# vymv/PupilOptixLab

Hardware: AMD Instinct MI355X
Metric: Mrays/sec + ms/frame, 1M-tri scene @1920x1080 8spp; 1/2/4/8-GPU scaling (higher is better)
Workload: dtype f32; 1 GPU; config4: 1,000,014-primitive sphere field (1,000,014 tris), 1920x1080, 8 spp, max_depth 4; rays_traced_plain_process=18645769168, parallelism=tiles32x1, area_emitters=2, accel=flat, emitter_select=guide, bvh_nodes=213019

## Files before the change

include/pupil_pt.h:

```cpp
#pragma once
#include <stddef.h>
#include <stdint.h>

#ifdef __cplusplus
extern "C" {
#endif

#define PUPIL_OK 0
#define PUPIL_ERR_INVALID -1
#define PUPIL_ERR_HIP -2
#define PUPIL_ERR_OOM -3
#define PUPIL_ERR_IO -4
#define PUPIL_ERR_UNSUPPORTED -5

#define PUPIL_TEX_RGB 0u
#define PUPIL_TEX_BITMAP 1u
#define PUPIL_TEX_CHECKERBOARD 2u

#define PUPIL_MAT_UNKNOWN 0u
#define PUPIL_MAT_DIFFUSE 1u
#define PUPIL_MAT_DIELECTRIC 2u
#define PUPIL_MAT_ROUGH_DIELECTRIC 3u
#define PUPIL_MAT_CONDUCTOR 4u
#define PUPIL_MAT_ROUGH_CONDUCTOR 5u
// ... 266 lines not shown
int pupil_debug_math(int device, uint32_t n, const float *x, const float *y2, float *out);
int pupil_debug_select_emitter(pupil_pt *pt, uint32_t n, const float *p, int32_t *out);
int pupil_debug_read_emitters(pupil_pt *pt, uint32_t first, uint32_t n, float *out);
int pupil_debug_emitter_sample(pupil_pt *pt, uint32_t emitter, uint32_t n, const float *xi, const float *pos_nrm,
                               float *out);
int pupil_debug_read_emitter_guide(pupil_pt *pt, uint32_t *bits, uint32_t *guide, uint32_t *inout_count);
int pupil_debug_shade_tables(pupil_pt *pt, uint32_t caps[4], uint32_t *fit);
int pupil_debug_env(pupil_pt *pt, uint32_t n, const float *xi_or_dir, const float *pos_nrm, uint32_t mode, float *out);
int pupil_debug_read_env_tables(pupil_pt *pt, uint32_t *width, uint32_t *height, float *col_cdf, float *row_cdf,
                                float *row_weight, float *normalization);
int pupil_debug_tex_sample(pupil_pt *pt, uint32_t material, uint32_t slot, uint32_t n, const float *uv, float *out);
int pupil_debug_read_material(pupil_pt *pt, uint32_t material, uint32_t *type, float out[3]);
int pupil_debug_fill_tlas_reserve(pupil_pt *pt, float value);
int pupil_debug_bvh_reinsert(int device, uint32_t n, const float *boxes, uint32_t rounds, double *cost,
                             uint32_t *kept, uint32_t *rejected);
int pupil_debug_partition(int device, uint32_t n, uint32_t capacity, const uint8_t *keys, uint32_t nbins,
                          uint32_t mode, uint32_t shift_or_tag, uint32_t bin_mask, const uint64_t *cum_in,
                          uint32_t *out, uint32_t *counts, uint32_t *starts, uint32_t *total, uint32_t *log,
                          uint64_t *cum_out, uint64_t *snap, uint32_t *info);

enum { PUPIL_IMAGE_AUTO = 0, PUPIL_IMAGE_EXR = 1, PUPIL_IMAGE_HDR = 2, PUPIL_IMAGE_PFM = 3 };
int pupil_image_save(const char *path, uint32_t width, uint32_t height, const float *rgba, uint32_t format);

int pupil_image_load(const char *path, uint32_t *width, uint32_t *height, float *rgba);

enum {
    PUPIL_DENOISE_USE_ALBEDO = 1,
    PUPIL_DENOISE_USE_NORMAL = 1 << 1,
    PUPIL_DENOISE_APPLY_TO_AOV = 1 << 2,
    PUPIL_DENOISE_USE_TEMPORAL = 1 << 3,
// ... 57 lines not shown
```

pupiloptixlab_amd/abi.py:

```python
from __future__ import annotations

import ctypes as C
import os

TEX_RGB, TEX_BITMAP, TEX_CHECKERBOARD = 0, 1, 2
MAT_UNKNOWN, MAT_DIFFUSE, MAT_DIELECTRIC, MAT_ROUGH_DIELECTRIC = 0, 1, 2, 3
MAT_CONDUCTOR, MAT_ROUGH_CONDUCTOR, MAT_PLASTIC, MAT_ROUGH_PLASTIC = 4, 5, 6, 7
EMITTER_NONE, EMITTER_TRI_AREA, EMITTER_SPHERE, EMITTER_CONST_ENV, EMITTER_ENV_MAP = 0, 1, 2, 3, 4
EMITTER_POINT, EMITTER_SPOT, EMITTER_DIRECTIONAL = 5, 6, 7
SHAPE_MESH, SHAPE_SPHERE = 0, 1

PUPIL_OK = OK = 0
ERR_INVALID, ERR_HIP, ERR_OOM, ERR_IO, ERR_UNSUPPORTED = -1, -2, -3, -4, -5
VERTS_DEVICE, VERTS_REBUILD = 1, 2
IMAGE_AUTO, IMAGE_EXR, IMAGE_HDR, IMAGE_PFM = 0, 1, 2, 3
ERR_NAMES = {-1: "PUPIL_ERR_INVALID", -2: "PUPIL_ERR_HIP", -3: "PUPIL_ERR_OOM", -4: "PUPIL_ERR_IO",
             -5: "PUPIL_ERR_UNSUPPORTED"}

f32p = C.POINTER(C.c_float)
u32p = C.POINTER(C.c_uint32)


class Texture(C.Structure):
    _fields_ = [("type", C.c_uint32), ("c0", C.c_float * 3), ("c1", C.c_float * 3),
# ... 155 lines not shown
                                           C.c_uint32, C.c_uint32, C.c_void_p]),
    "pupil_pt_query_rays": (C.c_int, [C.c_void_p, C.c_uint32, C.c_void_p, C.c_uint32, C.POINTER(RayHits), C.c_void_p]),
    "pupil_pt_query_camera": (C.c_int, [C.c_void_p, C.c_float, C.c_float, C.c_uint32, C.c_uint32, C.c_uint32,
                                         C.c_uint32, C.c_void_p, C.POINTER(RayHits), C.c_void_p]),
    "pupil_pt_query_info": (C.c_int, [C.c_void_p, C.POINTER(C.c_uint64), C.POINTER(C.c_uint64),
                                       C.POINTER(C.c_uint64), C.POINTER(C.c_double)]),
    "pupil_pt_radiance_rays": (C.c_int, [C.c_void_p, C.c_uint32, C.c_void_p, C.c_void_p, C.POINTER(Launch),
                                          C.POINTER(RayRadiance), C.c_void_p]),
    "pupil_pt_radiance_info": (C.c_int, [C.c_void_p, C.POINTER(C.c_uint64), C.POINTER(C.c_uint64),
                                          C.POINTER(C.c_uint64), C.POINTER(C.c_uint64), C.POINTER(C.c_uint64),
                                          C.POINTER(C.c_double)]),
    "pupil_pt_trace_rays": (C.c_int, [C.c_void_p, C.c_uint32, f32p, f32p, C.c_int]),
    "pupil_pt_export_bvh4": (C.c_int, [C.c_void_p, u32p, C.c_void_p, u32p, f32p, C.POINTER(C.c_int32)]),
    "pupil_debug_math": (C.c_int, [C.c_int, C.c_uint32, f32p, f32p, f32p]),
    "pupil_debug_bvh_reinsert": (C.c_int, [C.c_int, C.c_uint32, f32p, C.c_uint32, C.POINTER(C.c_double), u32p, u32p]),
    "pupil_debug_partition": (C.c_int, [C.c_int, C.c_uint32, C.c_uint32, C.POINTER(C.c_uint8), C.c_uint32, C.c_uint32,
                                         C.c_uint32, C.c_uint32, C.POINTER(C.c_uint64), u32p, u32p, u32p, u32p, u32p,
                                         C.POINTER(C.c_uint64), C.POINTER(C.c_uint64), u32p]),
    "pupil_image_save": (C.c_int, [C.c_char_p, C.c_uint32, C.c_uint32, f32p, C.c_uint32]),
    "pupil_debug_select_emitter": (C.c_int, [C.c_void_p, C.c_uint32, f32p, C.POINTER(C.c_int32)]),
    "pupil_debug_env": (C.c_int, [C.c_void_p, C.c_uint32, f32p, f32p, C.c_uint32, f32p]),
    "pupil_debug_emitter_sample": (C.c_int, [C.c_void_p, C.c_uint32, C.c_uint32, f32p, f32p, f32p]),
    "pupil_debug_tex_sample": (C.c_int, [C.c_void_p, C.c_uint32, C.c_uint32, C.c_uint32, f32p, f32p]),
    "pupil_image_load": (C.c_int, [C.c_char_p, C.POINTER(C.c_uint32), C.POINTER(C.c_uint32), f32p]),
    "pupil_world_create": (C.c_int, [C.POINTER(C.c_void_p)]),
    "pupil_world_load_xml": (C.c_int, [C.c_void_p, C.c_char_p]),
    "pupil_world_set_film": (C.c_int, [C.c_void_p, C.c_uint32, C.c_uint32, C.c_uint32]),
    "pupil_world_set_sensor": (C.c_int, [C.c_void_p, C.c_float, C.c_char, C.c_float, C.c_float, f32p]),
    "pupil_world_add_mesh": (C.c_int, [C.c_void_p, C.c_uint32, C.c_uint32, f32p, f32p, f32p, u32p, u32p]),
    "pupil_world_add_builtin_shape": (C.c_int, [C.c_void_p, C.c_char_p, u32p]),
# ... 72 lines not shown
```

pupiloptixlab_amd/csrc/bvh_build.hip:

```cpp
#include "bvh_build_detail.h"

#include <algorithm>
#include <cstdlib>
#include <cstring>

namespace pupil {

using namespace bvh;

namespace {

__global__ void k_prim_setup(BvhBuildInput in, float4 *recs, Aabb *boxes) {
    const uint32_t i = blockIdx.x * blockDim.x + threadIdx.x;
    if (i >= in.num_prims) return;
    const uint32_t inst_id = in.prim_inst[i];
    const DevInstance &inst = in.instances[inst_id];
    const uint32_t mtype = in.materials[inst.material].type;
    const uint32_t bin = (mtype >= 1u && mtype <= 7u) ? mtype : 8u;
    Aabb b;
    if (inst.kind == PUPIL_SHAPE_SPHERE) {
        const float *m = inst.to_world;
        const vec3 c = v3(m[3], m[7], m[11]);
        const float ex = sqrtf(m[0] * m[0] + m[1] * m[1] + m[2] * m[2]) * 1.001f;
        const float ey = sqrtf(m[4] * m[4] + m[5] * m[5] + m[6] * m[6]) * 1.001f;
// ... 90 lines not shown
__global__ void k_leaf_slots(Bvh4Node *nodes, uint32_t m, const unsigned long long *first_slot, uint32_t *slot) {
    const uint32_t j = blockIdx.x * blockDim.x + threadIdx.x;
    if (j >= m) return;
    Bvh4Node nd = nodes[j];
    for (int k = 0; k < 4; k++) {
        const int l = nd.child[k];
        if (l == kEmptyLink || l >= 0) continue;
        const uint32_t f = leaf_first(l), c = leaf_count(l), fs = (uint32_t)first_slot[f];
        for (uint32_t q = 0; q < c; q++) slot[f + q] = fs + q;
        nd.child[k] = make_leaf(fs, c);
    }
    nodes[j] = nd;
}

constexpr int kReinsDefault = 2;

BuildOptions read_build_options(uint32_t leaf_size) {
    BuildOptions o;
    const char *e = std::getenv("PUPIL_BVH_BUILDER");
    if (e && std::strcmp(e, "lbvh") == 0) o.builder = BuildOptions::Builder::Karras;
    e = std::getenv("PUPIL_BVH4_COLLAPSE");
    if (e && std::strcmp(e, "parity") == 0) o.collapse = BuildOptions::Collapse::Parity;
    else if (e && std::strcmp(e, "greedy") == 0) o.collapse = BuildOptions::Collapse::Greedy;
    o.sah_leaf = leaf_size;
    if ((e = std::getenv("PUPIL_SAH_LEAF"))) o.sah_leaf = (uint32_t)std::min(8, std::max((int)leaf_size, std::atoi(e)));
    o.reinsert_rounds = kReinsDefault;
    if ((e = std::getenv("PUPIL_BVH_REINSERT"))) o.reinsert_rounds = std::min(64, std::max(0, std::atoi(e)));
    o.reinsert_log = std::getenv("PUPIL_BVH_REINSERT_LOG") != nullptr;
    return o;
}

hipError_t leaf_slots_and_records(const BvhBuildInput &in, const uint32_t *order, const float4 *recs, bool leaf_root,
                                  BvhBuildOutput &out, hipStream_t s) {
    const uint32_t nrec = in.num_prims;
    const uint32_t g = (nrec + kBlock - 1) / kBlock;
    hipError_t err = hipSuccess;
    auto slot = scratch<uint32_t>(err, nrec);
    auto lsz = scratch<unsigned long long>(err, nrec);
    auto ssum = scratch<unsigned long long>(err, scan64_blocks((int)nrec));
    auto stot = scratch<unsigned long long>(err, 1);
    if (err) return err;
    const uint32_t m = leaf_root ? 0u : out.num_nodes4;
// ... 106 lines not shown
    float ms = 0.f;
    (void)hipEventElapsedTime(&ms, e0, e1);
    if (build_ms) *build_ms = ms;
    (void)hipEventDestroy(e0);
    (void)hipEventDestroy(e1);
    return err == hipSuccess ? 0 : -2;
}

int build_bvh4_over_boxes(const float *h_boxes, uint32_t n, std::vector<Bvh4Node> &nodes, std::vector<uint32_t> &order,
                          uint32_t *depth, hipStream_t s, int rounds, ReinsertLog *log) {
    if (n < 2) return -1;
    BuildOptions opts = read_build_options(1u);
    opts.builder = BuildOptions::Builder::Ploc;
    opts.collapse = BuildOptions::Collapse::Sah;
    if (rounds >= 0) opts.reinsert_rounds = rounds;
    const int m = (int)n;
    hipError_t err = hipSuccess;
    FrontEnd fe(err, m, false);
    Collapsed c4;
    if (!err) err = hipMemcpyAsync(fe.boxes.get(), h_boxes, sizeof(Aabb) * n, hipMemcpyHostToDevice, s);
    if (!err) {
        morton_order(fe, m, s);
        err = binary_tree(fe, m, opts, s, log);
    }
    if (!err) err = collapse_bvh4(fe.tree(m), 1u, opts, fe.spare_keys, fe.spare_vals, s, c4);
    if (!err) {
        nodes.resize(c4.num_nodes4);
        order.resize(n);
        err = hipMemcpyAsync(nodes.data(), c4.nodes4.get(), sizeof(Bvh4Node) * c4.num_nodes4, hipMemcpyDeviceToHost, s);
        if (!err) err = hipMemcpyAsync(order.data(), fe.sorted_vals, sizeof(uint32_t) * n, hipMemcpyDeviceToHost, s);
// ... 27 lines not shown
```

pupiloptixlab_amd/csrc/bvh_build_detail.h:

```cpp
#pragma once
#include <hip/hip_runtime.h>

#include <cstdint>
#include <vector>

#include "bvh4_quant.h"
#include "host/scoped_buffer.h"
#include "pt_kernels.h"

namespace pupil::bvh {

constexpr int kBlock = 256;
inline dim3 grid_for(int m) { return dim3((unsigned)((m + kBlock - 1) / kBlock)); }

struct Aabb {
    float lo[3];
    float hi[3];
};

__device__ __forceinline__ Aabb merge(const Aabb &a, const Aabb &b) {
    Aabb r;
    for (int k = 0; k < 3; k++) {
        r.lo[k] = fminf(a.lo[k], b.lo[k]);
        r.hi[k] = fmaxf(a.hi[k], b.hi[k]);
// ... 15 lines not shown

template <typename T>
DevBuf<T> scratch(hipError_t &err, size_t count) {
    DevBuf<T> b;
    if (!err) err = b.alloc(count);
    return b;
}

struct BuildOptions {
    enum class Builder { Ploc, Karras };
    enum class Collapse { Sah, Greedy, Parity };
    Builder builder = Builder::Ploc;
    Collapse collapse = Collapse::Sah;
    uint32_t sah_leaf = 0;
    int reinsert_rounds = 0;
    bool reinsert_log = false;
};

constexpr int kScanBlock = 1024;
constexpr int kScanItems = 4;
constexpr int kScanPer = kScanBlock * kScanItems;
inline int scan64_blocks(int n) { return (n + kScanPer - 1) / kScanPer; }
hipError_t scan64(unsigned long long *data, int n, unsigned long long *sums, unsigned long long *total,
                  hipStream_t s, unsigned long long *host_total = nullptr);

void scan32(uint32_t *data, uint32_t count, hipStream_t s);

struct BinaryTree;
struct FrontEnd {
    DevBuf<Aabb> boxes, node_boxes;
// ... 36 lines not shown
```

pupiloptixlab_amd/csrc/bvh_reinsert.hip:

```cpp
#include "bvh_build_detail.h"

#include <cstdio>

namespace pupil::bvh {

namespace {

constexpr int kReinsStack = 32;
constexpr int kReinsVisits = 256;

__device__ __forceinline__ int ref_u(int r, int nm1) { return r >= 0 ? r : nm1 + ~r; }
__device__ __forceinline__ int u_ref(int u, int nm1) { return u < nm1 ? u : ~(u - nm1); }

__global__ void k_reins_init(int n, const uint32_t *sorted_vals, const Aabb *prim_boxes, const int2 *node_child,
                             Aabb *box, int *parent) {
    const int i = blockIdx.x * blockDim.x + threadIdx.x;
    const int nm1 = n - 1;
    if (i < n) box[nm1 + i] = prim_boxes[sorted_vals[i]];
    if (i < nm1) {
        const int2 c = node_child[i];
        parent[ref_u(c.x, nm1)] = i;
        parent[ref_u(c.y, nm1)] = i;
        if (i == n - 2) parent[i] = -1;
    }
}

__global__ __launch_bounds__(kBlock) void k_reins_search(int n, const int2 *node_child, const Aabb *box,
                                                         const int *parent, int *cand_x, int *cand_pivot,
                                                         float *cand_gain, unsigned long long *claim) {
    const int u = blockIdx.x * blockDim.x + threadIdx.x;
    const int nm1 = n - 1, total = 2 * n - 1;
    if (u >= total) return;
    cand_x[u] = -1;
    const int P = parent[u];
    if (P < 0 || parent[P] < 0) return;
    const Aabb bl = box[u];
    const float al = half_area(bl);
    int st_node[kReinsStack];
    float st_ind[kReinsStack];
    float best = 0.f;
    int best_x = -1, best_pivot = -1;
    int visits = 0;
    int pivot = P, from = u;
    float bound = half_area(box[P]);
    Aabb shr;
    bool have_shr = false;
    while (visits < kReinsVisits) {
// ... 39 lines not shown
    if (best_x < 0) return;
    const int2 pc = node_child[P];
    const int S = ref_u(pc.x, nm1) == u ? ref_u(pc.y, nm1) : ref_u(pc.x, nm1);
    if (best_x == S) return;
    cand_x[u] = best_x;
    cand_pivot[u] = best_pivot;
    cand_gain[u] = best;
    const unsigned long long key = ((unsigned long long)__float_as_uint(best) << 32) | (unsigned)u;
    atomicMax(&claim[u], key);
    atomicMax(&claim[P], key);
    atomicMax(&claim[S], key);
    atomicMax(&claim[best_x], key);
    atomicMax(&claim[parent[best_x]], key);
}

__global__ void k_reins_resolve(int n, const int2 *node_child, const int *parent, const int *cand_x,
                                const float *cand_gain, const unsigned long long *claim, uint8_t *mover) {
    const int u = blockIdx.x * blockDim.x + threadIdx.x;
    const int nm1 = n - 1;
    if (u >= 2 * n - 1) return;
    const int X = cand_x[u];
    bool win = false;
    if (X >= 0) {
        const int P = parent[u];
        const int2 pc = node_child[P];
        const int S = ref_u(pc.x, nm1) == u ? ref_u(pc.y, nm1) : ref_u(pc.x, nm1);
        const unsigned long long key = ((unsigned long long)__float_as_uint(cand_gain[u]) << 32) | (unsigned)u;
        win = claim[u] == key && claim[P] == key && claim[S] == key && claim[X] == key && claim[parent[X]] == key;
    }
    mover[u] = win ? 1 : 0;
}

__global__ void k_reins_filter(int n, const int2 *node_child, const int *parent, const int *cand_x,
                               const int *cand_pivot, const uint8_t *mover, int3 *moves, int *num_moves) {
    const int u = blockIdx.x * blockDim.x + threadIdx.x;
    const int nm1 = n - 1;
    if (u >= 2 * n - 1 || !mover[u]) return;
    const int X = cand_x[u], pivot = cand_pivot[u];
    int a = parent[X];
    for (int k = 0; k < n && a >= 0 && a != pivot; k++) {
        if (mover[a]) return;
        a = parent[a];
    }
    const int P = parent[u], G = parent[P], XP = parent[X];
    const int sg = ref_u(node_child[G].x, nm1) == P ? 0 : 1;
    const int sx = ref_u(node_child[XP].x, nm1) == X ? 0 : 1;
    moves[atomicAdd(num_moves, 1)] = make_int3(u, sg, sx);
}

__global__ void k_reins_apply(int n, int num_moves, const int3 *moves, const int *cand_x, int2 *node_child,
                              int *parent) {
    const int k = blockIdx.x * blockDim.x + threadIdx.x;
    const int nm1 = n - 1;
    if (k >= num_moves) return;
    const int3 mv = moves[k];
    const int L = mv.x, X = cand_x[L];
    const int P = parent[L], G = parent[P], XP = parent[X];
    const int2 pc = node_child[P];
    const int S = ref_u(pc.x, nm1) == L ? ref_u(pc.y, nm1) : ref_u(pc.x, nm1);
    ((int *)&node_child[G])[mv.y] = u_ref(S, nm1);
    ((int *)&node_child[XP])[mv.z] = u_ref(P, nm1);
    node_child[P] = make_int2(u_ref(X, nm1), u_ref(L, nm1));
    parent[S] = G;
    parent[P] = XP;
    parent[X] = P;
}

__global__ void k_reins_refit(int n, const int2 *node_child, const int *parent, Aabb *box, int *node_count,
                              uint32_t *flags) {
    const int i = blockIdx.x * blockDim.x + threadIdx.x;
    const int nm1 = n - 1;
    if (i >= n) return;
    int node = parent[nm1 + i];
    for (int k = 0; k < n && node >= 0; k++) {
        __builtin_amdgcn_fence(__ATOMIC_RELEASE, "agent");
        const uint32_t prev = __hip_atomic_fetch_add(&flags[node], 1u, __ATOMIC_RELAXED, __HIP_MEMORY_SCOPE_AGENT);
        if (prev == 0u) return;
        __builtin_amdgcn_fence(__ATOMIC_ACQUIRE, "agent");
        const int2 c = node_child[node];
        box[node] = merge(box[ref_u(c.x, nm1)], box[ref_u(c.y, nm1)]);
        node_count[node] = (c.x >= 0 ? node_count[c.x] : 1) + (c.y >= 0 ? node_count[c.y] : 1);
        node = parent[node];
    }
}

__global__ __launch_bounds__(kBlock) void k_reins_cost(int m, const Aabb *box, double *partial) {
    __shared__ double sh[kBlock];
    const int i = blockIdx.x * kBlock + threadIdx.x;
    sh[threadIdx.x] = i < m ? (double)half_area(box[i]) : 0.0;
    __syncthreads();
    for (int o = kBlock / 2; o > 0; o >>= 1) {
        if ((int)threadIdx.x < o) sh[threadIdx.x] += sh[threadIdx.x + o];
        __syncthreads();
    }
    if (threadIdx.x == 0) partial[blockIdx.x] = sh[0];
}

struct ReinsertScratch {
    DevBuf<int2> w_child;
    DevBuf<Aabb> w_box;
    DevBuf<int> w_count, parent, cand_x, cand_pivot;
    DevBuf<float> cand_gain;
    DevBuf<unsigned long long> claim;
    DevBuf<uint8_t> mover;
    DevBuf<int3> moves;
    DevBuf<int> num_moves;
    DevBuf<uint32_t> flags;
    DevBuf<double> partial;
    std::vector<double> host_partial;

    ReinsertScratch(hipError_t &err, int n) {
        const int total = 2 * n - 1, nblk = (n - 1 + kBlock - 1) / kBlock;
        w_child = scratch<int2>(err, n);
        w_box = scratch<Aabb>(err, total);
        w_count = scratch<int>(err, n);
        parent = scratch<int>(err, total);
        cand_x = scratch<int>(err, total);
        cand_pivot = scratch<int>(err, total);
        cand_gain = scratch<float>(err, total);
        claim = scratch<unsigned long long>(err, total);
        mover = scratch<uint8_t>(err, total);
        moves = scratch<int3>(err, total);
        num_moves = scratch<int>(err, 1);
        flags = scratch<uint32_t>(err, n);
        partial = scratch<double>(err, nblk);
        host_partial.resize((size_t)nblk);
    }

    hipError_t cost(int n, hipStream_t s, double *out) {
        const int nblk = (int)host_partial.size();
        hipLaunchKernelGGL(k_reins_cost, dim3(nblk), dim3(kBlock), 0, s, n - 1, w_box.get(), partial.get());
        hipError_t e = hipMemcpyAsync(host_partial.data(), partial.get(), sizeof(double) * nblk, hipMemcpyDeviceToHost, s);
        if (!e) e = hipStreamSynchronize(s);
        double c = 0.0;
        for (double v : host_partial) c += v;
        *out = c;
        return e;
    }

    hipError_t round(int n, hipStream_t s, bool *moved, double *after) {
        const int total = 2 * n - 1;
        *moved = false;
        hipError_t err = hipMemsetAsync(claim.get(), 0, sizeof(unsigned long long) * total, s);
        if (!err) err = hipMemsetAsync(num_moves.get(), 0, sizeof(int), s);
        if (err) return err;
        hipLaunchKernelGGL(k_reins_search, grid_for(total), dim3(kBlock), 0, s, n, w_child.get(), w_box.get(),
                           parent.get(), cand_x.get(), cand_pivot.get(), cand_gain.get(), claim.get());
        hipLaunchKernelGGL(k_reins_resolve, grid_for(total), dim3(kBlock), 0, s, n, w_child.get(), parent.get(),
                           cand_x.get(), cand_gain.get(), claim.get(), mover.get());
        hipLaunchKernelGGL(k_reins_filter, grid_for(total), dim3(kBlock), 0, s, n, w_child.get(), parent.get(),
                           cand_x.get(), cand_pivot.get(), mover.get(), moves.get(), num_moves.get());
        int nmoves = 0;
        err = hipMemcpyAsync(&nmoves, num_moves.get(), sizeof(int), hipMemcpyDeviceToHost, s);
        if (!err) err = hipStreamSynchronize(s);
        if (err || nmoves <= 0) return err;
        hipLaunchKernelGGL(k_reins_apply, grid_for(nmoves), dim3(kBlock), 0, s, n, nmoves, moves.get(), cand_x.get(),
                           w_child.get(), parent.get());
        err = hipMemsetAsync(flags.get(), 0, sizeof(uint32_t) * n, s);
        if (err) return err;
        hipLaunchKernelGGL(k_reins_refit, grid_for(n), dim3(kBlock), 0, s, n, w_child.get(), parent.get(), w_box.get(),
                           w_count.get(), flags.get());
        *moved = true;
        return cost(n, s, after);
    }
};

}

hipError_t reinsert_ploc(int n, const BuildOptions &opts, const uint32_t *vals_in, const Aabb *prim_boxes,
                         int2 *node_child, Aabb *node_box, int *node_count, ReinsertLog *log, hipStream_t s) {
    const int rounds = opts.reinsert_rounds;
    ReinsertLog env_log;
    const bool print = !log && rounds > 0 && opts.reinsert_log;
    if (print) log = &env_log;
    if (log) *log = ReinsertLog{};
    if (n < 2 || (rounds <= 0 && !log)) return hipSuccess;
    const int nm1 = n - 1;
    hipError_t err = hipSuccess;
    ReinsertScratch w(err, n);
    if (err) {
        (void)hipGetLastError();
        return err == hipErrorOutOfMemory ? hipSuccess : err;
    }
    double cost = 0.0;
    err = hipMemcpyAsync(w.w_child.get(), node_child, sizeof(int2) * nm1, hipMemcpyDeviceToDevice, s);
    if (!err) err = hipMemcpyAsync(w.w_box.get(), node_box, sizeof(Aabb) * nm1, hipMemcpyDeviceToDevice, s);
    if (!err) err = hipMemcpyAsync(w.w_count.get(), node_count, sizeof(int) * nm1, hipMemcpyDeviceToDevice, s);
    if (!err) {
        hipLaunchKernelGGL(k_reins_init, grid_for(n), dim3(kBlock), 0, s, n, vals_in, prim_boxes, w.w_child.get(),
                           w.w_box.get(), w.parent.get());
        err = w.cost(n, s, &cost);
    }
    if (!err && log) log->costs.push_back(cost);
    for (int r = 0; r < rounds && !err; r++) {
        bool moved = false;
        double after = 0.0;
        err = w.round(n, s, &moved, &after);
        if (err || !moved) break;
        if (after > cost) {
            if (log) log->rejected++;
            break;
        }
        err = hipMemcpyAsync(node_child, w.w_child.get(), sizeof(int2) * nm1, hipMemcpyDeviceToDevice, s);
        if (!err) err = hipMemcpyAsync(node_box, w.w_box.get(), sizeof(Aabb) * nm1, hipMemcpyDeviceToDevice, s);
        if (!err) err = hipMemcpyAsync(node_count, w.w_count.get(), sizeof(int) * nm1, hipMemcpyDeviceToDevice, s);
        cost = after;
        if (!err && log) {
            log->costs.push_back(cost);
            log->kept++;
        }
    }
    if (!err) err = hipStreamSynchronize(s);
    if (print && !log->costs.empty())
        std::fprintf(stderr, "reinsert: %d leaves, %d rounds asked, %d kept, %d rejected, cost %.9g -> %.9g\n", n, rounds,
                     log->kept, log->rejected, log->costs.front(), log->costs.back());
    return err;
}

}
```

pupiloptixlab_amd/csrc/engine.hip:

```cpp
#include <hip/hip_runtime.h>

#include <algorithm>
#include <chrono>
#include <cmath>
#include <cstddef>
#include <cstdio>
#include <cstdlib>
#include <cstring>
#include <string>
#include <vector>

#include "host/emitter_weight.h"
#include "host/instance_record.h"
#include "host/pipe_schedule.h"
#include "host/prim_tables.h"
#include "host/scoped_buffer.h"
#include "pt_accel.h"

namespace {

thread_local std::string g_last_error;

constexpr uint32_t kMaxPairs = 4096;

// ... 2419 lines not shown
    if (!pt) return fail(PUPIL_ERR_INVALID, "null argument");
    if (!pt->accel.two_level) return fail(PUPIL_ERR_UNSUPPORTED, "the flattened BVH has no TLAS reserve");
    HIP_TRY(hipSetDevice(pt->device));
    HIP_TRY(order_after_renders(pt));
    const uint64_t lo = pt->accel.tl.tlas_nodes, hi = std::min<uint64_t>(pt->accel.tl.tlas_cap, pt->accel.nodes4_count());
    if (hi > lo) {
        std::vector<float> junk((hi - lo) * (sizeof(Bvh4Node) / sizeof(float)), value);
        HIP_TRY(hipMemcpyAsync((void *)(pt->sc.nodes4 + lo), junk.data(), sizeof(float) * junk.size(),
                               hipMemcpyHostToDevice, pt->own_stream));
        HIP_TRY(hipStreamSynchronize(pt->own_stream));
    }
    if (const int rc = pt->accel.publish()) return rc;
    return derive_cull_set(pt);
}

int pupil_debug_bvh_reinsert(int device, uint32_t n, const float *boxes, uint32_t rounds, double *cost,
                             uint32_t *kept, uint32_t *rejected) {
    if (!boxes || !cost) return fail(PUPIL_ERR_INVALID, "null argument");
    if (n < 2 || rounds > 64u) return fail(PUPIL_ERR_INVALID, "needs n >= 2 boxes and at most 64 rounds");
    HIP_TRY(hipSetDevice(device));
    std::vector<Bvh4Node> nodes;
    std::vector<uint32_t> order;
    ReinsertLog log;
    if (build_bvh4_over_boxes(boxes, n, nodes, order, nullptr, nullptr, (int)rounds, &log) != 0)
        return fail(PUPIL_ERR_HIP, "the box BVH build failed");
    if (log.costs.empty()) return fail(PUPIL_ERR_HIP, "out of device memory for the reinsertion pass");
    for (uint32_t r = 0; r <= rounds; r++) cost[r] = log.costs[std::min<size_t>(r, log.costs.size() - 1)];
    if (kept) *kept = (uint32_t)log.kept;
    if (rejected) *rejected = (uint32_t)log.rejected;
    return PUPIL_OK;
}

int pupil_debug_partition(int device, uint32_t n, uint32_t capacity, const uint8_t *keys, uint32_t nbins,
                          uint32_t mode, uint32_t shift_or_tag, uint32_t bin_mask, const uint64_t *cum_in,
                          uint32_t *out, uint32_t *counts, uint32_t *starts, uint32_t *total, uint32_t *log,
                          uint64_t *cum_out, uint64_t *snap, uint32_t *info) {
    if ((!keys && n > 0) || !out || !counts || !starts) return fail(PUPIL_ERR_INVALID, "null argument");
    if (nbins < 1u || nbins > (uint32_t)kPartMaxBins) return fail(PUPIL_ERR_INVALID, "nbins must be in 1..9");
    if (mode > 1u) return fail(PUPIL_ERR_INVALID, "mode must be 0 (exclusive) or 1 (flags)");
    if (mode == 1u && nbins != 2u) return fail(PUPIL_ERR_INVALID, "the flags mode has two bins");
    if (n > capacity) return fail(PUPIL_ERR_INVALID, "n exceeds the capacity");
    if (capacity > (1u << 28)) return fail(PUPIL_ERR_INVALID, "the capacity exceeds 2^28 paths");
    if (!cum_in && (cum_out || snap)) return fail(PUPIL_ERR_INVALID, "cum_out and snap need cum_in");
    HIP_TRY(hipSetDevice(device));
    constexpr uint32_t kFill = 0xA5A5A5A5u, kGuard = 64;
// ... 67 lines not shown
```

pupiloptixlab_amd/csrc/pt_kernels.h:

```cpp
#pragma once

#include <vector>

#include <hip/hip_runtime.h>

#include "pt_scene.h"
#include "host/instance_record.h"

namespace pupil {

constexpr int kTraceBlock = 128;
constexpr int kTraceWavesPerSimd = 7;
constexpr int kTraceWavesPerSimdTL = 5;
constexpr int kStackOvf = 160;
constexpr int kRing = 16;
constexpr int kTraceStackEntries = kRing + kStackOvf;
constexpr int kShadeBlock = 256;
constexpr uint32_t kShadeMaxBlocks = 16384;
constexpr uint32_t kMaxDepth = 128;
constexpr uint32_t kNumQueues = 9;
constexpr uint32_t kMissIndex = 0xFFFFFFFFu;

struct PathState {
    float4 *ray_o;
// ... 275 lines not shown
    uint32_t num_records = 0;
    std::vector<uint32_t> level_start;
};
int build_lbvh(const BvhBuildInput &in, BvhBuildOutput &out, uint32_t leaf_size, hipStream_t s, double *build_ms,
               bool force_lbvh = false);
int build_bvh_bounded(const BvhBuildInput &in, BvhBuildOutput &out, uint32_t leaf_size, hipStream_t s,
                      double *build_ms, uint32_t reserve);
void free_lbvh(BvhBuildOutput &out);
int refit_bvh4(const BvhBuildInput &in, BvhBuildOutput &out, const uint8_t *moved, float *nbox, hipStream_t s,
               double *ms, bool records_only = false);
void launch_refit_levels(Bvh4Node *nodes, const std::vector<uint32_t> &level_start, uint32_t node_base,
                         const float4 *recs, float *nbox, hipStream_t s);
void launch_refresh_attrs(const BvhBuildInput &in, const BvhBuildOutput &out, const uint8_t *moved, hipStream_t s);
void launch_refresh_attrs_shape(float4 *attrs, uint32_t n, const float *positions, const float *normals,
                                const uint32_t *indices, hipStream_t s);
struct ReinsertLog {
    std::vector<double> costs;
    int kept = 0;
    int rejected = 0;
};
int build_bvh4_over_boxes(const float *h_boxes, uint32_t n, std::vector<Bvh4Node> &nodes,
                          std::vector<uint32_t> &order, uint32_t *depth, hipStream_t s, int rounds = -1,
                          ReinsertLog *log = nullptr);

}
```

Baseline: 8122 Mrays/s.

## Run BVH reinsertion rounds on device with gated undo and incremental refit

Moves the per-round cost check of the BVH reinsertion pass onto the GPU, using a gate kernel and a device-side state struct. This removes the per-round host synchronizations and copies. Rejected rounds are undone on the device from recorded back-pointers, and refit now walks only the ancestors of moved nodes instead of the whole tree. It adds an optional convergence threshold and debug hooks; the change affects BVH build time, not steady-state trace throughput.

```diff
diff --git a/include/pupil_pt.h b/include/pupil_pt.h
--- a/include/pupil_pt.h
+++ b/include/pupil_pt.h
@@ -304,6 +304,9 @@
 int pupil_debug_fill_tlas_reserve(pupil_pt *pt, float value);
 int pupil_debug_bvh_reinsert(int device, uint32_t n, const float *boxes, uint32_t rounds, double *cost,
                              uint32_t *kept, uint32_t *rejected);
+int pupil_debug_bvh_reinsert_tree(int device, uint32_t n, const float *boxes, uint32_t rounds, double threshold,
+                                  uint32_t flags, int32_t reject_round, double *cost, uint32_t *kept,
+                                  uint32_t *rejected, int32_t *child, float *box, int32_t *count, int32_t *parent);
 int pupil_debug_partition(int device, uint32_t n, uint32_t capacity, const uint8_t *keys, uint32_t nbins,
                           uint32_t mode, uint32_t shift_or_tag, uint32_t bin_mask, const uint64_t *cum_in,
                           uint32_t *out, uint32_t *counts, uint32_t *starts, uint32_t *total, uint32_t *log,
diff --git a/pupiloptixlab_amd/abi.py b/pupiloptixlab_amd/abi.py
--- a/pupiloptixlab_amd/abi.py
+++ b/pupiloptixlab_amd/abi.py
@@ -193,6 +193,9 @@
     "pupil_pt_export_bvh4": (C.c_int, [C.c_void_p, u32p, C.c_void_p, u32p, f32p, C.POINTER(C.c_int32)]),
     "pupil_debug_math": (C.c_int, [C.c_int, C.c_uint32, f32p, f32p, f32p]),
     "pupil_debug_bvh_reinsert": (C.c_int, [C.c_int, C.c_uint32, f32p, C.c_uint32, C.POINTER(C.c_double), u32p, u32p]),
+    "pupil_debug_bvh_reinsert_tree": (C.c_int, [C.c_int, C.c_uint32, f32p, C.c_uint32, C.c_double, C.c_uint32,
+                                                 C.c_int32, C.POINTER(C.c_double), u32p, u32p, C.POINTER(C.c_int32),
+                                                 f32p, C.POINTER(C.c_int32), C.POINTER(C.c_int32)]),
     "pupil_debug_partition": (C.c_int, [C.c_int, C.c_uint32, C.c_uint32, C.POINTER(C.c_uint8), C.c_uint32, C.c_uint32,
                                          C.c_uint32, C.c_uint32, C.POINTER(C.c_uint64), u32p, u32p, u32p, u32p, u32p,
                                          C.POINTER(C.c_uint64), C.POINTER(C.c_uint64), u32p]),
diff --git a/pupiloptixlab_amd/csrc/bvh_build.hip b/pupiloptixlab_amd/csrc/bvh_build.hip
--- a/pupiloptixlab_amd/csrc/bvh_build.hip
+++ b/pupiloptixlab_amd/csrc/bvh_build.hip
@@ -128,6 +128,7 @@
 }
 
 constexpr int kReinsDefault = 2;
+constexpr double kReinsThreshold = 0.0;
 
 BuildOptions read_build_options(uint32_t leaf_size) {
     BuildOptions o;
@@ -140,6 +141,8 @@
     if ((e = std::getenv("PUPIL_SAH_LEAF"))) o.sah_leaf = (uint32_t)std::min(8, std::max((int)leaf_size, std::atoi(e)));
     o.reinsert_rounds = kReinsDefault;
     if ((e = std::getenv("PUPIL_BVH_REINSERT"))) o.reinsert_rounds = std::min(64, std::max(0, std::atoi(e)));
+    o.reinsert_threshold = kReinsThreshold;
+    if ((e = std::getenv("PUPIL_BVH_REINSERT_EPS"))) o.reinsert_threshold = std::min(1.0, std::max(0.0, std::atof(e)));
     o.reinsert_log = std::getenv("PUPIL_BVH_REINSERT_LOG") != nullptr;
     return o;
 }
@@ -276,6 +279,7 @@
     opts.builder = BuildOptions::Builder::Ploc;
     opts.collapse = BuildOptions::Collapse::Sah;
     if (rounds >= 0) opts.reinsert_rounds = rounds;
+    if (log && log->ask.threshold >= 0.0) opts.reinsert_threshold = log->ask.threshold;
     const int m = (int)n;
     hipError_t err = hipSuccess;
     FrontEnd fe(err, m, false);
diff --git a/pupiloptixlab_amd/csrc/bvh_build_detail.h b/pupiloptixlab_amd/csrc/bvh_build_detail.h
--- a/pupiloptixlab_amd/csrc/bvh_build_detail.h
+++ b/pupiloptixlab_amd/csrc/bvh_build_detail.h
@@ -53,6 +53,7 @@
     Collapse collapse = Collapse::Sah;
     uint32_t sah_leaf = 0;
     int reinsert_rounds = 0;
+    double reinsert_threshold = 0.0;
     bool reinsert_log = false;
 };
 
diff --git a/pupiloptixlab_amd/csrc/bvh_reinsert.hip b/pupiloptixlab_amd/csrc/bvh_reinsert.hip
--- a/pupiloptixlab_amd/csrc/bvh_reinsert.hip
+++ b/pupiloptixlab_amd/csrc/bvh_reinsert.hip
@@ -1,5 +1,6 @@
 #include "bvh_build_detail.h"
 
+#include <algorithm>
 #include <cstdio>
 
 namespace pupil::bvh {
@@ -8,6 +9,17 @@
 
 constexpr int kReinsStack = 32;
 constexpr int kReinsVisits = 256;
+constexpr int kReinsMaxRounds = 64;
+constexpr int kReinsMoveBlocks = 1024;
+
+struct ReinsState {
+    double cost;
+    int stop;
+    int kept;
+    int rejected;
+    int undo;
+    double costs[kReinsMaxRounds + 1];
+};
 
 __device__ __forceinline__ int ref_u(int r, int nm1) { return r >= 0 ? r : nm1 + ~r; }
 __device__ __forceinline__ int u_ref(int u, int nm1) { return u < nm1 ? u : ~(u - nm1); }
@@ -25,12 +37,13 @@
     }
 }
 
-__global__ __launch_bounds__(kBlock) void k_reins_search(int n, const int2 *node_child, const Aabb *box,
-                                                         const int *parent, int *cand_x, int *cand_pivot,
-                                                         float *cand_gain, unsigned long long *claim) {
+__global__ __launch_bounds__(kBlock) void k_reins_search(int n, const ReinsState *st, const int2 *node_child,
+                                                         const Aabb *box, const int *parent, int *cand_x,
+                                                         int *cand_pivot, float *cand_gain,
+                                                         unsigned long long *claim) {
     const int u = blockIdx.x * blockDim.x + threadIdx.x;
     const int nm1 = n - 1, total = 2 * n - 1;
-    if (u >= total) return;
+    if (u >= total || st->stop) return;
     cand_x[u] = -1;
     const int P = parent[u];
     if (P < 0 || parent[P] < 0) return;
@@ -100,11 +113,12 @@
     atomicMax(&claim[parent[best_x]], key);
 }
 
-__global__ void k_reins_resolve(int n, const int2 *node_child, const int *parent, const int *cand_x,
-                                const float *cand_gain, const unsigned long long *claim, uint8_t *mover) {
+__global__ void k_reins_resolve(int n, const ReinsState *st, const int2 *node_child, const int *parent,
+                                const int *cand_x, const float *cand_gain, const unsigned long long *claim,
+                                uint8_t *mover) {
     const int u = blockIdx.x * blockDim.x + threadIdx.x;
     const int nm1 = n - 1;
-    if (u >= 2 * n - 1) return;
+    if (u >= 2 * n - 1 || st->stop) return;
     const int X = cand_x[u];
     bool win = false;
     if (X >= 0) {
@@ -117,11 +131,14 @@
     mover[u] = win ? 1 : 0;
 }
 
-__global__ void k_reins_filter(int n, const int2 *node_child, const int *parent, const int *cand_x,
-                               const int *cand_pivot, const uint8_t *mover, int3 *moves, int *num_moves) {
+__global__ void k_reins_filter(int n, const ReinsState *st, const int2 *node_child, const int *parent,
+                               const int *cand_x, const int *cand_pivot, const uint8_t *mover,
+                               unsigned long long *claim, int3 *moves, int *num_moves) {
     const int u = blockIdx.x * blockDim.x + threadIdx.x;
     const int nm1 = n - 1;
-    if (u >= 2 * n - 1 || !mover[u]) return;
+    if (u >= 2 * n - 1 || st->stop) return;
+    claim[u] = 0ull;
+    if (!mover[u]) return;
     const int X = cand_x[u], pivot = cand_pivot[u];
     int a = parent[X];
     for (int k = 0; k < n && a >= 0 && a != pivot; k++) {
@@ -134,29 +151,110 @@
     moves[atomicAdd(num_moves, 1)] = make_int3(u, sg, sx);
 }
 
-__global__ void k_reins_apply(int n, int num_moves, const int3 *moves, const int *cand_x, int2 *node_child,
-                              int *parent) {
-    const int k = blockIdx.x * blockDim.x + threadIdx.x;
-    const int nm1 = n - 1;
-    if (k >= num_moves) return;
-    const int3 mv = moves[k];
-    const int L = mv.x, X = cand_x[L];
-    const int P = parent[L], G = parent[P], XP = parent[X];
-    const int2 pc = node_child[P];
-    const int S = ref_u(pc.x, nm1) == L ? ref_u(pc.y, nm1) : ref_u(pc.x, nm1);
-    ((int *)&node_child[G])[mv.y] = u_ref(S, nm1);
-    ((int *)&node_child[XP])[mv.z] = u_ref(P, nm1);
-    node_child[P] = make_int2(u_ref(X, nm1), u_ref(L, nm1));
-    parent[S] = G;
-    parent[P] = XP;
-    parent[X] = P;
-}
-
-__global__ void k_reins_refit(int n, const int2 *node_child, const int *parent, Aabb *box, int *node_count,
-                              uint32_t *flags) {
+__global__ void k_reins_apply(int n, const ReinsState *st, const int *num_moves, const int3 *moves,
+                              const int *cand_x, int2 *node_child, int *parent, int4 *back) {
+    const int nm1 = n - 1;
+    if (st->stop) return;
+    const int count = *num_moves;
+    for (int k = blockIdx.x * blockDim.x + threadIdx.x; k < count; k += gridDim.x * blockDim.x) {
+        const int3 mv = moves[k];
+        const int L = mv.x, X = cand_x[L];
+        const int P = parent[L], G = parent[P], XP = parent[X];
+        const int2 pc = node_child[P];
+        const int ls = ref_u(pc.x, nm1) == L ? 0 : 1;
+        const int S = ls == 0 ? ref_u(pc.y, nm1) : ref_u(pc.x, nm1);
+        ((int *)&node_child[G])[mv.y] = u_ref(S, nm1);
+        ((int *)&node_child[XP])[mv.z] = u_ref(P, nm1);
+        node_child[P] = make_int2(u_ref(X, nm1), u_ref(L, nm1));
+        parent[S] = G;
+        parent[P] = XP;
+        parent[X] = P;
+        back[k] = make_int4(G, S, XP, ls);
+    }
+}
+
+__global__ void k_reins_undo(int n, const ReinsState *st, const int *num_moves, const int3 *moves, const int4 *back,
+                             int2 *node_child, int *parent) {
+    const int nm1 = n - 1;
+    if (st->undo < 0) return;
+    const int count = num_moves[st->undo];
+    for (int k = blockIdx.x * blockDim.x + threadIdx.x; k < count; k += gridDim.x * blockDim.x) {
+        const int3 mv = moves[k];
+        const int4 b = back[k];
+        const int L = mv.x, G = b.x, S = b.y, XP = b.z;
+        const int P = parent[L], X = ref_u(node_child[P].x, nm1);
+        ((int *)&node_child[G])[mv.y] = u_ref(P, nm1);
+        ((int *)&node_child[XP])[mv.z] = u_ref(X, nm1);
+        node_child[P] = b.w == 0 ? make_int2(u_ref(L, nm1), u_ref(S, nm1)) : make_int2(u_ref(S, nm1), u_ref(L, nm1));
+        parent[S] = P;
+        parent[P] = G;
+        parent[X] = XP;
+    }
+}
+
+__device__ __forceinline__ int2 reins_starts(int k, bool undo, const int3 *moves, const int4 *back,
+                                             const int *parent) {
+    const int P = parent[moves[k].x];
+    const int4 b = back[k];
+    return undo ? make_int2(P, b.z) : make_int2(b.x, P);
+}
+
+__device__ __forceinline__ bool reins_phase(const ReinsState *st, bool undo, const int *num_moves, int *count) {
+    if (undo ? st->undo < 0 : st->stop != 0) return false;
+    *count = undo ? num_moves[st->undo] : num_moves[0];
+    return true;
+}
+
+__global__ void k_reins_mark(int n, const ReinsState *st, bool undo, const int *num_moves, const int3 *moves,
+                             const int4 *back, const int *parent, uint32_t *dirty, uint32_t *pending) {
+    int count = 0;
+    if (!reins_phase(st, undo, num_moves, &count)) return;
+    for (int k = blockIdx.x * blockDim.x + threadIdx.x; k < count; k += gridDim.x * blockDim.x) {
+        const int2 s = reins_starts(k, undo, moves, back, parent);
+        for (int e = 0; e < 2; e++) {
+            int node = e == 0 ? s.x : s.y;
+            atomicAdd(&pending[node], 1u);
+            for (int j = 0; j < n; j++) {
+                if (atomicExch(&dirty[node], 1u) != 0u) break;
+                node = parent[node];
+                if (node < 0) break;
+                atomicAdd(&pending[node], 1u);
+            }
+        }
+    }
+}
+
+__global__ void k_reins_refit_dirty(int n, const ReinsState *st, bool undo, const int *num_moves, const int3 *moves,
+                                    const int4 *back, const int2 *node_child, const int *parent, Aabb *box,
+                                    int *node_count, uint32_t *dirty, uint32_t *pending) {
+    const int nm1 = n - 1;
+    int count = 0;
+    if (!reins_phase(st, undo, num_moves, &count)) return;
+    for (int k = blockIdx.x * blockDim.x + threadIdx.x; k < count; k += gridDim.x * blockDim.x) {
+        const int2 s = reins_starts(k, undo, moves, back, parent);
+        for (int e = 0; e < 2; e++) {
+            int node = e == 0 ? s.x : s.y;
+            for (int j = 0; j < n && node >= 0; j++) {
+                __builtin_amdgcn_fence(__ATOMIC_RELEASE, "agent");
+                const uint32_t prev =
+                    __hip_atomic_fetch_sub(&pending[node], 1u, __ATOMIC_RELAXED, __HIP_MEMORY_SCOPE_AGENT);
+                if (prev != 1u) break;
+                __builtin_amdgcn_fence(__ATOMIC_ACQUIRE, "agent");
+                const int2 c = node_child[node];
+                box[node] = merge(box[ref_u(c.x, nm1)], box[ref_u(c.y, nm1)]);
+                node_count[node] = (c.x >= 0 ? node_count[c.x] : 1) + (c.y >= 0 ? node_count[c.y] : 1);
+                dirty[node] = 0u;
+                node = parent[node];
+            }
+        }
+    }
+}
+
+__global__ void k_reins_refit(int n, const ReinsState *st, const int2 *node_child, const int *parent, Aabb *box,
+                              int *node_count, uint32_t *flags) {
     const int i = blockIdx.x * blockDim.x + threadIdx.x;
     const int nm1 = n - 1;
-    if (i >= n) return;
+    if (i >= n || st->stop) return;
     int node = parent[nm1 + i];
     for (int k = 0; k < n && node >= 0; k++) {
         __builtin_amdgcn_fence(__ATOMIC_RELEASE, "agent");
@@ -170,8 +268,10 @@
     }
 }
 
-__global__ __launch_bounds__(kBlock) void k_reins_cost(int m, const Aabb *box, double *partial) {
+__global__ __launch_bounds__(kBlock) void k_reins_cost(int m, const ReinsState *st, const Aabb *box,
+                                                       double *partial) {
     __shared__ double sh[kBlock];
+    if (st->stop) return;
     const int i = blockIdx.x * kBlock + threadIdx.x;
     sh[threadIdx.x] = i < m ? (double)half_area(box[i]) : 0.0;
     __syncthreads();
@@ -180,6 +280,45 @@
         __syncthreads();
     }
     if (threadIdx.x == 0) partial[blockIdx.x] = sh[0];
+}
+
+__global__ __launch_bounds__(kBlock) void k_reins_gate(int nblk, const double *partial, int round,
+                                                       const int *num_moves, double threshold, int reject_round,
+                                                       ReinsState *st) {
+    __shared__ double sh[kBlock];
+    if (st->stop) return;
+    double c = 0.0;
+    for (int base = 0; base < nblk; base += kBlock) {
+        const int i = base + (int)threadIdx.x;
+        sh[threadIdx.x] = i < nblk ? partial[i] : 0.0;
+        __syncthreads();
+        if (threadIdx.x == 0) {
+            const int m = nblk - base < kBlock ? nblk - base : kBlock;
+            for (int j = 0; j < m; j++) c += sh[j];
+        }
+        __syncthreads();
+    }
+    if (threadIdx.x != 0) return;
+    if (round < 0) {
+        st->cost = c;
+        st->costs[0] = c;
+        st->undo = -1;
+        return;
+    }
+    if (*num_moves <= 0) {
+        st->stop = 1;
+        return;
+    }
+    const double before = st->cost;
+    if (c > before || round == reject_round) {
+        st->rejected++;
+        st->undo = round;
+        st->stop = 1;
+        return;
+    }
+    st->cost = c;
+    st->costs[++st->kept] = c;
+    if (before - c < threshold * before) st->stop = 1;
 }
 
 struct ReinsertScratch {
@@ -190,13 +329,17 @@
     DevBuf<unsigned long long> claim;
     DevBuf<uint8_t> mover;
     DevBuf<int3> moves;
+    DevBuf<int4> back;
     DevBuf<int> num_moves;
+    DevBuf<uint32_t> marks;
     DevBuf<uint32_t> flags;
     DevBuf<double> partial;
-    std::vector<double> host_partial;
-
-    ReinsertScratch(hipError_t &err, int n) {
-        const int total = 2 * n - 1, nblk = (n - 1 + kBlock - 1) / kBlock;
+    DevBuf<ReinsState> state;
+    int nblk = 0;
+
+    ReinsertScratch(hipError_t &err, int n, bool full_refit) {
+        const int total = 2 * n - 1;
+        nblk = (n - 1 + kBlock - 1) / kBlock;
         w_child = scratch<int2>(err, n);
         w_box = scratch<Aabb>(err, total);
         w_count = scratch<int>(err, n);
@@ -207,47 +350,53 @@
         claim = scratch<unsigned long long>(err, total);
         mover = scratch<uint8_t>(err, total);
         moves = scratch<int3>(err, total);
-        num_moves = scratch<int>(err, 1);
-        flags = scratch<uint32_t>(err, n);
+        back = scratch<int4>(err, total);
+        num_moves = scratch<int>(err, kReinsMaxRounds);
+        marks = scratch<uint32_t>(err, 2 * (size_t)n);
+        if (full_refit) flags = scratch<uint32_t>(err, n);
         partial = scratch<double>(err, nblk);
-        host_partial.resize((size_t)nblk);
-    }
-
-    hipError_t cost(int n, hipStream_t s, double *out) {
-        const int nblk = (int)host_partial.size();
-        hipLaunchKernelGGL(k_reins_cost, dim3(nblk), dim3(kBlock), 0, s, n - 1, w_box.get(), partial.get());
-        hipError_t e = hipMemcpyAsync(host_partial.data(), partial.get(), sizeof(double) * nblk, hipMemcpyDeviceToHost, s);
-        if (!e) e = hipStreamSynchronize(s);
-        double c = 0.0;
-        for (double v : host_partial) c += v;
-        *out = c;
-        return e;
-    }
-
-    hipError_t round(int n, hipStream_t s, bool *moved, double *after) {
+        state = scratch<ReinsState>(err, 1);
+    }
+
+    uint32_t *dirty() { return marks.get(); }
+    uint32_t *pending(int n) { return marks.get() + n; }
+    dim3 move_grid(int n) const { return dim3((unsigned)std::min(kReinsMoveBlocks, (2 * n - 1 + kBlock - 1) / kBlock)); }
+
+    void cost_and_gate(int n, hipStream_t s, int round, double threshold, int reject_round) {
+        hipLaunchKernelGGL(k_reins_cost, dim3(nblk), dim3(kBlock), 0, s, n - 1, state.get(), w_box.get(), partial.get());
+        hipLaunchKernelGGL(k_reins_gate, dim3(1), dim3(kBlock), 0, s, nblk, partial.get(), round,
+                           num_moves.get() + std::max(round, 0), threshold, reject_round, state.get());
+    }
+
+    void refit_marked(int n, hipStream_t s, bool undo, const int *count) {
+        hipLaunchKernelGGL(k_reins_mark, move_grid(n), dim3(kBlock), 0, s, n, state.get(), undo, count, moves.get(),
+                           back.get(), parent.get(), dirty(), pending(n));
+        hipLaunchKernelGGL(k_reins_refit_dirty, move_grid(n), dim3(kBlock), 0, s, n, state.get(), undo, count,
+                           moves.get(), back.get(), w_child.get(), parent.get(), w_box.get(), w_count.get(), dirty(),
+                           pending(n));
+    }
+
+    hipError_t round(int n, int r, const BuildOptions &opts, const ReinsertAsk &ask, hipStream_t s) {
         const int total = 2 * n - 1;
-        *moved = false;
-        hipError_t err = hipMemsetAsync(claim.get(), 0, sizeof(unsigned long long) * total, s);
-        if (!err) err = hipMemsetAsync(num_moves.get(), 0, sizeof(int), s);
-        if (err) return err;
-        hipLaunchKernelGGL(k_reins_search, grid_for(total), dim3(kBlock), 0, s, n, w_child.get(), w_box.get(),
-                           parent.get(), cand_x.get(), cand_pivot.get(), cand_gain.get(), claim.get());
-        hipLaunchKernelGGL(k_reins_resolve, grid_for(total), dim3(kBlock), 0, s, n, w_child.get(), parent.get(),
-                           cand_x.get(), cand_gain.get(), claim.get(), mover.get());
-        hipLaunchKernelGGL(k_reins_filter, grid_for(total), dim3(kBlock), 0, s, n, w_child.get(), parent.get(),
-                           cand_x.get(), cand_pivot.get(), mover.get(), moves.get(), num_moves.get());
-        int nmoves = 0;
-        err = hipMemcpyAsync(&nmoves, num_moves.get(), sizeof(int), hipMemcpyDeviceToHost, s);
-        if (!err) err = hipStreamSynchronize(s);
-        if (err || nmoves <= 0) return err;
-        hipLaunchKernelGGL(k_reins_apply, grid_for(nmoves), dim3(kBlock), 0, s, n, nmoves, moves.get(), cand_x.get(),
-                           w_child.get(), parent.get());
-        err = hipMemsetAsync(flags.get(), 0, sizeof(uint32_t) * n, s);
-        if (err) return err;
-        hipLaunchKernelGGL(k_reins_refit, grid_for(n), dim3(kBlock), 0, s, n, w_child.get(), parent.get(), w_box.get(),
-                           w_count.get(), flags.get());
-        *moved = true;
-        return cost(n, s, after);
+        int *count = num_moves.get() + r;
+        hipLaunchKernelGGL(k_reins_search, grid_for(total), dim3(kBlock), 0, s, n, state.get(), w_child.get(),
+                           w_box.get(), parent.get(), cand_x.get(), cand_pivot.get(), cand_gain.get(), claim.get());
+        hipLaunchKernelGGL(k_reins_resolve, grid_for(total), dim3(kBlock), 0, s, n, state.get(), w_child.get(),
+                           parent.get(), cand_x.get(), cand_gain.get(), claim.get(), mover.get());
+        hipLaunchKernelGGL(k_reins_filter, grid_for(total), dim3(kBlock), 0, s, n, state.get(), w_child.get(),
+                           parent.get(), cand_x.get(), cand_pivot.get(), mover.get(), claim.get(), moves.get(), count);
+        hipLaunchKernelGGL(k_reins_apply, move_grid(n), dim3(kBlock), 0, s, n, state.get(), count, moves.get(),
+                           cand_x.get(), w_child.get(), parent.get(), back.get());
+        if (ask.full_refit) {
+            const hipError_t err = hipMemsetAsync(flags.get(), 0, sizeof(uint32_t) * n, s);
+            if (err) return err;
+            hipLaunchKernelGGL(k_reins_refit, grid_for(n), dim3(kBlock), 0, s, n, state.get(), w_child.get(),
+                               parent.get(), w_box.get(), w_count.get(), flags.get());
+        } else {
+            refit_marked(n, s, false, count);
+        }
+        cost_and_gate(n, s, r, opts.reinsert_threshold, ask.reject_round);
+        return hipGetLastError();
     }
 };
 
@@ -255,48 +404,62 @@
 
 hipError_t reinsert_ploc(int n, const BuildOptions &opts, const uint32_t *vals_in, const Aabb *prim_boxes,
                          int2 *node_child, Aabb *node_box, int *node_count, ReinsertLog *log, hipStream_t s) {
-    const int rounds = opts.reinsert_rounds;
+    const int rounds = std::min(opts.reinsert_rounds, kReinsMaxRounds);
     ReinsertLog env_log;
     const bool print = !log && rounds > 0 && opts.reinsert_log;
     if (print) log = &env_log;
-    if (log) *log = ReinsertLog{};
+    const ReinsertAsk ask = log ? log->ask : ReinsertAsk{};
+    if (log) {
+        *log = ReinsertLog{};
+        log->ask = ask;
+    }
     if (n < 2 || (rounds <= 0 && !log)) return hipSuccess;
-    const int nm1 = n - 1;
+    const int nm1 = n - 1, total = 2 * n - 1;
     hipError_t err = hipSuccess;
-    ReinsertScratch w(err, n);
+    ReinsertScratch w(err, n, ask.full_refit);
     if (err) {
         (void)hipGetLastError();
         return err == hipErrorOutOfMemory ? hipSuccess : err;
     }
-    double cost = 0.0;
     err = hipMemcpyAsync(w.w_child.get(), node_child, sizeof(int2) * nm1, hipMemcpyDeviceToDevice, s);
     if (!err) err = hipMemcpyAsync(w.w_box.get(), node_box, sizeof(Aabb) * nm1, hipMemcpyDeviceToDevice, s);
     if (!err) err = hipMemcpyAsync(w.w_count.get(), node_count, sizeof(int) * nm1, hipMemcpyDeviceToDevice, s);
+    if (!err) err = hipMemsetAsync(w.state.get(), 0, sizeof(ReinsState), s);
+    if (!err) err = hipMemsetAsync(w.num_moves.get(), 0, sizeof(int) * kReinsMaxRounds, s);
+    if (!err) err = hipMemsetAsync(w.claim.get(), 0, sizeof(unsigned long long) * total, s);
+    if (!err) err = hipMemsetAsync(w.marks.get(), 0, sizeof(uint32_t) * 2 * (size_t)n, s);
     if (!err) {
         hipLaunchKernelGGL(k_reins_init, grid_for(n), dim3(kBlock), 0, s, n, vals_in, prim_boxes, w.w_child.get(),
                            w.w_box.get(), w.parent.get());
-        err = w.cost(n, s, &cost);
-    }
-    if (!err && log) log->costs.push_back(cost);
-    for (int r = 0; r < rounds && !err; r++) {
-        bool moved = false;
-        double after = 0.0;
-        err = w.round(n, s, &moved, &after);
-        if (err || !moved) break;
-        if (after > cost) {
-            if (log) log->rejected++;
-            break;
-        }
+        w.cost_and_gate(n, s, -1, 0.0, -1);
+    }
+    for (int r = 0; r < rounds && !err; r++) err = w.round(n, r, opts, ask, s);
+    if (!err && rounds > 0) {
+        hipLaunchKernelGGL(k_reins_undo, w.move_grid(n), dim3(kBlock), 0, s, n, w.state.get(), w.num_moves.get(),
+                           w.moves.get(), w.back.get(), w.w_child.get(), w.parent.get());
+        w.refit_marked(n, s, true, w.num_moves.get());
         err = hipMemcpyAsync(node_child, w.w_child.get(), sizeof(int2) * nm1, hipMemcpyDeviceToDevice, s);
         if (!err) err = hipMemcpyAsync(node_box, w.w_box.get(), sizeof(Aabb) * nm1, hipMemcpyDeviceToDevice, s);
         if (!err) err = hipMemcpyAsync(node_count, w.w_count.get(), sizeof(int) * nm1, hipMemcpyDeviceToDevice, s);
-        cost = after;
-        if (!err && log) {
-            log->costs.push_back(cost);
-            log->kept++;
-        }
+    }
+    ReinsState st{};
+    if (!err && log) err = hipMemcpyAsync(&st, w.state.get(), sizeof(st), hipMemcpyDeviceToHost, s);
+    if (!err && log && ask.want_tree) {
+        log->child.resize(2 * (size_t)nm1);
+        log->box.resize(6 * (size_t)total);
+        log->count.resize((size_t)nm1);
+        log->parent.resize((size_t)total);
+        err = hipMemcpyAsync(log->child.data(), w.w_child.get(), sizeof(int2) * nm1, hipMemcpyDeviceToHost, s);
+        if (!err) err = hipMemcpyAsync(log->box.data(), w.w_box.get(), sizeof(Aabb) * total, hipMemcpyDeviceToHost, s);
+        if (!err) err = hipMemcpyAsync(log->count.data(), w.w_count.get(), sizeof(int) * nm1, hipMemcpyDeviceToHost, s);
+        if (!err) err = hipMemcpyAsync(log->parent.data(), w.parent.get(), sizeof(int) * total, hipMemcpyDeviceToHost, s);
     }
     if (!err) err = hipStreamSynchronize(s);
+    if (!err && log) {
+        log->kept = st.kept;
+        log->rejected = st.rejected;
+        log->costs.assign(st.costs, st.costs + st.kept + 1);
+    }
     if (print && !log->costs.empty())
         std::fprintf(stderr, "reinsert: %d leaves, %d rounds asked, %d kept, %d rejected, cost %.9g -> %.9g\n", n, rounds,
                      log->kept, log->rejected, log->costs.front(), log->costs.back());
diff --git a/pupiloptixlab_amd/csrc/engine.hip b/pupiloptixlab_amd/csrc/engine.hip
--- a/pupiloptixlab_amd/csrc/engine.hip
+++ b/pupiloptixlab_amd/csrc/engine.hip
@@ -2457,21 +2457,37 @@
     return derive_cull_set(pt);
 }
 
-int pupil_debug_bvh_reinsert(int device, uint32_t n, const float *boxes, uint32_t rounds, double *cost,
-                             uint32_t *kept, uint32_t *rejected) {
+int pupil_debug_bvh_reinsert_tree(int device, uint32_t n, const float *boxes, uint32_t rounds, double threshold,
+                                  uint32_t flags, int32_t reject_round, double *cost, uint32_t *kept,
+                                  uint32_t *rejected, int32_t *child, float *box, int32_t *count, int32_t *parent) {
     if (!boxes || !cost) return fail(PUPIL_ERR_INVALID, "null argument");
     if (n < 2 || rounds > 64u) return fail(PUPIL_ERR_INVALID, "needs n >= 2 boxes and at most 64 rounds");
+    if (!(threshold >= 0.0)) return fail(PUPIL_ERR_INVALID, "the threshold must be >= 0");
     HIP_TRY(hipSetDevice(device));
     std::vector<Bvh4Node> nodes;
     std::vector<uint32_t> order;
     ReinsertLog log;
+    log.ask.threshold = threshold;
+    log.ask.full_refit = (flags & 1u) != 0;
+    log.ask.reject_round = reject_round;
+    log.ask.want_tree = child || box || count || parent;
     if (build_bvh4_over_boxes(boxes, n, nodes, order, nullptr, nullptr, (int)rounds, &log) != 0)
         return fail(PUPIL_ERR_HIP, "the box BVH build failed");
     if (log.costs.empty()) return fail(PUPIL_ERR_HIP, "out of device memory for the reinsertion pass");
     for (uint32_t r = 0; r <= rounds; r++) cost[r] = log.costs[std::min<size_t>(r, log.costs.size() - 1)];
     if (kept) *kept = (uint32_t)log.kept;
     if (rejected) *rejected = (uint32_t)log.rejected;
-    return PUPIL_OK;
+    if (child) std::copy(log.child.begin(), log.child.end(), child);
+    if (box) std::copy(log.box.begin(), log.box.end(), box);
+    if (count) std::copy(log.count.begin(), log.count.end(), count);
+    if (parent) std::copy(log.parent.begin(), log.parent.end(), parent);
+    return PUPIL_OK;
+}
+
+int pupil_debug_bvh_reinsert(int device, uint32_t n, const float *boxes, uint32_t rounds, double *cost,
+                             uint32_t *kept, uint32_t *rejected) {
+    return pupil_debug_bvh_reinsert_tree(device, n, boxes, rounds, 0.0, 0u, -1, cost, kept, rejected, nullptr, nullptr,
+                                         nullptr, nullptr);
 }
 
 int pupil_debug_partition(int device, uint32_t n, uint32_t capacity, const uint8_t *keys, uint32_t nbins,
diff --git a/pupiloptixlab_amd/csrc/pt_kernels.h b/pupiloptixlab_amd/csrc/pt_kernels.h
--- a/pupiloptixlab_amd/csrc/pt_kernels.h
+++ b/pupiloptixlab_amd/csrc/pt_kernels.h
@@ -313,10 +313,19 @@
 void launch_refresh_attrs(const BvhBuildInput &in, const BvhBuildOutput &out, const uint8_t *moved, hipStream_t s);
 void launch_refresh_attrs_shape(float4 *attrs, uint32_t n, const float *positions, const float *normals,
                                 const uint32_t *indices, hipStream_t s);
+struct ReinsertAsk {
+    double threshold = -1.0;
+    bool full_refit = false;
+    int reject_round = -1;
+    bool want_tree = false;
+};
 struct ReinsertLog {
+    ReinsertAsk ask;
     std::vector<double> costs;
     int kept = 0;
     int rejected = 0;
+    std::vector<int> child, count, parent;
+    std::vector<float> box;
 };
 int build_bvh4_over_boxes(const float *h_boxes, uint32_t n, std::vector<Bvh4Node> &nodes,
                           std::vector<uint32_t> &order, uint32_t *depth, hipStream_t s, int rounds = -1,
```

New measurement: 8118 Mrays/s, median of 2. No clear change (-0.0%).
